# PhilippBongartz/RepeatResolver

Measured on AMD Instinct MI355X. Metric: sum-of-pairs DP cells/sec, higher is better.
Workload: dtype u32

## Files before the change

repeatresolver_amd/csrc/pwr_device.hip:

```cpp
#include <hip/hip_runtime.h>

#include <algorithm>
#include <chrono>
#include <cstdint>
#include <cstdio>
#include <cstdlib>
#include <cstring>
#include <new>
#include <thread>
#include <type_traits>
#include <vector>

#include "pwr.h"

#define PWR_INF 0x40000000u
#define PWR_BIG 0x7fffffff

struct Hdr {
    int W;
    int nslots;
    int nfree;
    int cur;
    int status;
    int stop;
// ... 193 lines not shown
}

template <int NT>
__device__ __forceinline__ unsigned block_incl_add(unsigned v, unsigned *sh, unsigned &total)
{
    const int lane = threadIdx.x & 63, wave = threadIdx.x >> 6;
    unsigned incl = wave_incl_add(v);
    if (lane == 63) sh[wave] = incl;
    __syncthreads();
    unsigned wp = 0, tot = 0;
#pragma unroll
    for (int w = 0; w < NT / 64; ++w) {
        unsigned s = sh[w];
        wp += (w < wave) ? s : 0u;
        tot += s;
    }
    __syncthreads();
    total = tot;
    return incl + wp;
}

template <int NT>
__device__ __forceinline__ unsigned block_min_u32(unsigned v, unsigned *sh)
{
    for (int o = 32; o > 0; o >>= 1) v = min(v, (unsigned)__shfl_xor((int)v, o));
    if ((threadIdx.x & 63) == 0) sh[threadIdx.x >> 6] = v;
    __syncthreads();
    unsigned r = 0xffffffffu;
#pragma unroll
    for (int w = 0; w < NT / 64; ++w) r = min(r, sh[w]);
    __syncthreads();
    return r;
}
template <int NT>
__device__ __forceinline__ int block_max_i32(int v, int *sh)
{
    for (int o = 32; o > 0; o >>= 1) v = max(v, __shfl_xor(v, o));
    if ((threadIdx.x & 63) == 0) sh[threadIdx.x >> 6] = v;
    __syncthreads();
    int r = INT_MIN;
#pragma unroll
    for (int w = 0; w < NT / 64; ++w) r = max(r, sh[w]);
    __syncthreads();
    return r;
}

__device__ __forceinline__ const int *cur_order(const DState &st)
{
    return st.hdr->cur ? st.order1 : st.order0;
}

#define GATHER_NT 1024
#define GATHER_G 16
struct GatherPart { unsigned long long ucost, cells; unsigned sum4, maxS, lastcov, tag; };

__device__ __forceinline__ int gather_row_of(const Hdr *hd, const int *bplan, int job, int *boff_out)
{
    int boff = 0;
    if (bplan[0] && job < PLAN_MAX) boff = bplan[1 + job];
    else {
        const unsigned long long ah = hd->ahead;
        int cnt = -1;
        for (boff = 0; boff < 64; ++boff) if (!((ah >> boff) & 1ull) && ++cnt == job) break;
        if (boff == 64) boff = 64 + (job - cnt - 1);
    }
    *boff_out = boff;
    const int kk = hd->next_row + boff;
    if (hd->status != 0 || hd->need_grow || job >= hd->nb || kk >= hd->row_end) return -1;
    return kk;
}

__global__ __launch_bounds__(GATHER_NT) void k_gather_a(DState st, JobBufs jb, const int *jobrows)
{
    const int job = blockIdx.x, g = blockIdx.y, tid = threadIdx.x;
    JobMeta *m = &jb.meta[job];
    const Hdr *hd = st.hdr;
    int boff;
    const int kk = gather_row_of(hd, st.bplan, job, &boff);
    if (g == 0) {
        const int nj = (int)gridDim.x;
        if (tid == 0) { CommitJob z; z.nchg = z.nev = z.ndel = 0; z.first = 0x7fffffff; z.u0 = z.u1 = 0; z.scanned = 0; z.pad = 0; jb.cjob[job] = z; jb.chkdone[job] = 0; }
        for (int j = tid; j < nj; j += GATHER_NT) { jb.pair_cf[(size_t)job * nj + j] = 0; jb.pair_left[(size_t)job * nj + j] = 0; }
    }
    if (kk < 0) { if (tid == 0 && g == 0) m->active = 0; return; }
    const int k = jobrows[kk];
    const int L = st.rowlen[k];
    const int W = hd->W;
    if (L == 0) {
        if (tid == 0 && g == 0) { m->k = k; m->L = 0; m->ok = 1; m->W = W; m->nnew = 0; m->cells = 0; m->ver = hd->version; m->active = 1; m->off = boff; m->wide = 0; m->abort = 0; }
        return;
    }
    const long long off = st.rowoff[k];
    const int *order = cur_order(st);
    int *way = jb.way + (size_t)job * jb.Lmax;
    const int B = st.B, H = st.H;
    const int way0 = st.rank[st.pos[off]], wayL = st.rank[st.pos[off + L - 1]];
    const int a0 = max(0, way0 - H), aL = max(0, wayL - H);
    const int lo = max(0, a0 - 1), hi = min(W - 1, aL + B - 1);
    const int n = hi - lo + 1;
    if (g == 0 && tid < 64 && hd->jumpmask != 0ull) {
        bool bad = false;
        if (tid > boff && ((hd->jumpmask >> tid) & 1ull)) {
            const int kkj = hd->next_row + tid;
            const int kj = jobrows[kkj], Lj = st.rowlen[kj];
            const long long oj = st.rowoff[kj];
            const int f = st.rank[st.pos[oj]], l = st.rank[st.pos[oj + Lj - 1]];
            const int *rec = st.bplan + JR_BASE + 4 * (kkj & 63);
            const int es = (int)((unsigned)hd->events_total - (unsigned)rec[0]);
            bad = !(hi + 2 < f - rec[1] - es || l + rec[2] + es < lo - 2);
        }
        if (__ballot(bad) != 0ull && tid == 0) atomicCAS(&st.hdr->status, 0, PWR_ERR_ORDER);
    }
    const int x0 = (int)((long long)L * g / GATHER_G), x1 = (int)((long long)L * (g + 1) / GATHER_G);
    uint8_t *mark = jb.mark + (size_t)job * jb.colcap;
    const int c0 = g == 0 ? lo : st.rank[st.pos[off + min(x0, L - 1)]], c1 = (g == GATHER_G - 1 || x1 >= L) ? hi + 1 : st.rank[st.pos[off + x1]];
    (void)n;
    for (int i = c0 - lo + tid; i < c1 - lo; i += GATHER_NT) mark[i] = 0;
    __syncthreads();
    unsigned long long mycells = 0;
    uint4 *desc = jb.desc + (size_t)job * jb.Lmax;
    const int NWg = jb.wpNW, MSg = jb.wpMS;
// ... 253 lines not shown
    unsigned carry = s_carry, maxS = 0;
    if (tid == 0) s_cov[0] = s_covl;
    __syncthreads();
    int it2 = 0;
    for (int base = i0; base < i1; base += GATHER_NT, ++it2) {
        const int i = base + tid;
        const bool valid = i < i1;
        const int y = lo + i;
        uint32_t w[6] = {0, 0, 0, 0, 0, 0};
        if (it2 < GC_K) {
#pragma unroll
            for (int k = 0; k < GC_K; ++k)
                if (it2 == k) {
#pragma unroll
                    for (int b = 0; b < 6; ++b) w[b] = cw[k][b];
                }
        } else if (valid) tally_of(y, w, &ucost);
        unsigned tot;
        const unsigned gin = block_incl_add<GATHER_NT>(w[4], sh, tot);
        s_cov[tid + 1] = w[5];
        __syncthreads();
        const unsigned covl = s_cov[tid];
        __syncthreads();
        if (tid == GATHER_NT - 1) s_cov[0] = w[5];
        if (valid) {
            const unsigned upc = (y == 0 || y == W - 1) ? PWR_INF : max(w[5], covl);
            const int gq = (int)(carry + gin);
            rec2[2 * i] = make_int4((int)w[0] - gq, (int)w[1] - gq, (int)w[2] - gq, (int)w[3] - gq);
            rec2[2 * i + 1] = make_int4((int)(upc == PWR_INF ? PWR_INF - 1u : upc) - gq, gq, (int)PWR_INF - gq, 0);
            maxS = max(maxS, max(max(w[0], w[1]), max(max(w[2], w[3]), max(w[4], w[5]))));
        }
        carry += tot;
        __syncthreads();
    }
    const unsigned mx = (unsigned)(~block_min_u32<GATHER_NT>(~maxS, sh));
    for (int o = 32; o > 0; o >>= 1) ucost += __shfl_xor(ucost, o);
    if ((tid & 63) == 0) s_u[tid >> 6] = ucost;
    __syncthreads();
    if (tid == 0) {
        unsigned long long U = 0;
        for (int w = 0; w < GATHER_NT / 64; ++w) U += s_u[w];
        __hip_atomic_store(&part[g].ucost, U, __ATOMIC_RELAXED, __HIP_MEMORY_SCOPE_AGENT);
        __hip_atomic_store(&part[g].maxS, mx, __ATOMIC_RELAXED, __HIP_MEMORY_SCOPE_AGENT);
        __hip_atomic_store(&part[g].lastcov, tag, __ATOMIC_RELEASE, __HIP_MEMORY_SCOPE_AGENT);
    }
    if (g == GATHER_G - 1 && tid < 64) {
        unsigned long long Ut = 0, cs = 0;
        unsigned mxt = 0;
        if (tid < GATHER_G) {
            while (__hip_atomic_load(&part[tid].lastcov, __ATOMIC_ACQUIRE, __HIP_MEMORY_SCOPE_AGENT) != tag) __builtin_amdgcn_s_sleep(1);
            Ut = __hip_atomic_load(&part[tid].ucost, __ATOMIC_RELAXED, __HIP_MEMORY_SCOPE_AGENT);
            mxt = __hip_atomic_load(&part[tid].maxS, __ATOMIC_RELAXED, __HIP_MEMORY_SCOPE_AGENT);
            cs = part[tid].cells;
        }
        for (int o = 32; o > 0; o >>= 1) { Ut += __shfl_xor(Ut, o); cs += __shfl_xor(cs, o); mxt = max(mxt, (unsigned)__shfl_xor((int)mxt, o)); }
        if (tid == 0) {
            const unsigned long long bound = Ut + (unsigned long long)mxt * (unsigned long long)(2 * B + 4096);
            m->maxS = mxt; m->cells = cs;
            m->wide = (jb.force64 || !(bound < (unsigned long long)PWR_INF && carry < (1u << 29))) ? 1 : 0;
            if (m->wide) st.hdr->need64 = 65;
        }
    }
}

#define V2_D 128
#define V2_PD 512
#define V2_R 64
#define V2_SPINS 256
#define FBIG 0x3fffffff
#define UNI(v) __builtin_amdgcn_readfirstlane(v)

__device__ __forceinline__ unsigned acc_push(unsigned acc, unsigned long long mask)
{
    unsigned long long carry_out;
    asm("v_addc_co_u32_e64 %0, %1, %0, %0, %2" : "+v"(acc), "=s"(carry_out) : "s"(mask));
    return acc;
}
#define ICMP_SGE 39
#define ICMP_SLE 41

#define V2_LOAD(MSX, SLOT, AU, AG, AI, GL)                                                       \
    {                                                                                            \
        _Pragma("unroll") for (int i = 0; i < C; ++i) {                                          \
            const int y_ = lo + (MSX) * MS + lc + i;                                             \
            int4 p_ = make_int4(PWR_BIG / 2, PWR_BIG / 2, PWR_BIG / 2, PWR_BIG / 2);             \
            int4 q_ = make_int4(PWR_BIG / 2, 0, PWR_BIG / 2, 0);                                 \
            if (y_ <= hi) { p_ = rec2[2 * (y_ - lo)]; q_ = rec2[2 * (y_ - lo) + 1]; }            \
            ldsS[wave][SLOT][0][lc + i] = p_.x; ldsS[wave][SLOT][1][lc + i] = p_.y;              \
            ldsS[wave][SLOT][2][lc + i] = p_.z; ldsS[wave][SLOT][3][lc + i] = p_.w;              \
            AU[i] = q_.x; AG[i] = q_.y; AI[i] = q_.z;                                            \
        }                                                                                        \
        const int yq_ = lo + (MSX) * MS - 1;                                                     \
        GL = (yq_ >= lo && yq_ <= hi) ? UNI(rec2[2 * (yq_ - lo) + 1].y) : 0;                     \
    }

template <int NW, int C>
__global__ __launch_bounds__(NW * 64) void k_fill_v2(DState st, JobBufs jb)
{
    constexpr int MS = 64 * C, RS = NW * MS;
    constexpr int MBDUMP = NW * V2_D, PTDUMP = V2_PD;
    __shared__ unsigned long long mbQ[2 * (MBDUMP + NW * 64)];
    __shared__ unsigned long long ptQ[PTDUMP + NW * 64];
    __shared__ __attribute__((aligned(16))) int ldsS[NW][2][4][MS];
    __shared__ int rdone[NW];
    __shared__ int s_done;
#define LD64(REF) __hip_atomic_load(&(REF), __ATOMIC_RELAXED, __HIP_MEMORY_SCOPE_WORKGROUP)
// ... 2753 lines not shown
#define HIPC(call)                                                                     \
    do {                                                                               \
        hipError_t e_ = (call);                                                        \
        if (e_ != hipSuccess) {                                                        \
            fprintf(stderr, "pwr: %s failed: %s\n", #call, hipGetErrorString(e_));    \
            return PWR_ERR_DEVICE;                                                     \
        }                                                                              \
    } while (0)

struct pwr_ctx {
    int T = 0, B = 0, H = 0, device = 0;
    int W_host = 0;
    std::vector<unsigned char> text;
    bool on_device = false;
    DState st{};
    JobBufs jb{};
    int njobs = 0;
    int *d_jobrows = nullptr;
    int *d_rowids = nullptr;
    std::vector<int> ids, pos_lo;
    unsigned long long *d_score = nullptr;
    hipStream_t stream = nullptr;
    std::vector<int> rowlen;
    long long sumL = 0;
    int Lmax = 0;
    int window = 3;
    double batch_ema = 1.0;
    int profile = 0;
    unsigned gather_tag = 0;
    int force64 = 0;
    int evcap = EVCAP;
    int stall_test = 0;
    int par_trace = 2;
    int cap_slack = 8192;
    int spec_len = 6;
    int fill_mode = 4;
    double host_enqueue_s = 0, host_wait_s = 0;
    unsigned host_seq = 0;
    int seen_fallback = 0, seen_need64 = 0;
    unsigned trace_epoch = 0;
    unsigned fill_epoch = 0;
    int wave_cols = 0;
    int wp_waves = 5;
    int one_wg = 0;
    int one_wg_lds = 0;
    int fill_lds = 0;
    int seg_rows = 160;
    int seg_align = 16;
    int seg_max = 64;
    int seg_budget = 0;
    int seg_minrows = 64;
    int spec_inorder = 64, plan_gate_rel = 1, plan_len = 0;
    int check_in_trace = 1;
    int fail_stops = 1, hard_rows = 1, hard_up_pm = 300, hard_down_pm = 0;
    int plan_slack = PLAN_SLACK, plan_evrate_x100 = (int)(PLAN_EVRATE_MAX * 100.0f);
    int plan_ahead = 1;
    int seg_balance = 0;
    int split_rank = 0, split_world = 1;
    int split_k0 = 0, split_kend = 0;
    int src_start = 1;
    int warm_pct = 190;
    int warm_adapt = 1;
    int warm_min_pct = 100;
    int warm_down_pm = 5, warm_up_pm = 50;
    pwr_stats stats{};
    std::vector<std::pair<hipEvent_t, hipEvent_t>> ev_pool;
    size_t ev_used = 0;
    void *h_hdr = nullptr;
    void *h_ring = nullptr;
    unsigned char *snap_dev = nullptr, *snap_host = nullptr;
    size_t snap_cap = 0;
    hipStream_t snap_stream = nullptr;
    hipEvent_t snap_taken = nullptr, snap_done = nullptr;
    bool snap_busy = false;
    std::vector<void *> allocs;
};
struct pwr_snapshot { pwr_ctx *c; int rows, width; size_t bytes; };

template <class F>
static void par_rows(int T, F f)
{
    unsigned nt = std::min<unsigned>(std::max(1u, std::thread::hardware_concurrency()), 16u);
    nt = (unsigned)std::max(1, std::min<int>((int)nt, T / 64));
    if (nt <= 1) { f(0, T, 0); return; }
    std::vector<std::thread> th;
    for (unsigned t = 0; t < nt; ++t)
        th.emplace_back([=]() { f((int)((long long)T * t / nt), (int)((long long)T * (t + 1) / nt), (int)t); });
    for (auto &x : th) x.join();
}
static unsigned par_threads(int T)
{
    unsigned nt = std::min<unsigned>(std::max(1u, std::thread::hardware_concurrency()), 16u);
    return (unsigned)std::max(1, std::min<int>((int)nt, T / 64));
}

static int code_of_char(unsigned char c)
{
    switch (c) {
    case 'a': case 'A': return 0;
    case 'c': case 'C': return 1;
    case 'g': case 'G': return 2;
    case 't': case 'T': return 3;
    case '-': case '_': return 4;
    case ' ': return 5;
    default: return -1;
    }
// ... 503 lines not shown
static int drain_events(pwr_ctx *c)
{
    if (!c->ev_used) return PWR_OK;
    HIPC(hipStreamSynchronize(c->stream));
    for (size_t i = 0; i < c->ev_used; ++i) {
        float ms = 0;
        HIPC(hipEventElapsedTime(&ms, c->ev_pool[i].first, c->ev_pool[i].second));
        c->stats.fill_ms += ms;
    }
    c->ev_used = 0;
    return PWR_OK;
}

static int ensure_device(pwr_ctx *c)
{
    if (c->on_device) { if (hipSetDevice(c->device) != hipSuccess) return PWR_ERR_DEVICE; return PWR_OK; }
    int rc = upload(c);
    if (rc) { free_device(c); return rc; }
    return PWR_OK;
}

static void stats_from_hdr(pwr_ctx *c, const Hdr &h)
{
    c->stats.cells_computed = h.cells_computed;
    c->stats.cells_reference = h.cells_reference;
    c->stats.rows_changed = h.rows_changed;
    c->stats.batches = h.batches;
    c->stats.rows_committed = h.rows_committed;
    c->stats.rows_recomputed = h.rows_recomputed;
    c->stats.rows_wide = h.rows_wide;
    c->stats.stalls = h.stalls;
    c->stats.rows_ahead = h.rows_ahead;
    c->stats.seg_jobs = h.seg_jobs; c->stats.segs = h.segs; c->stats.seg_fails = h.seg_fails;
    c->stats.rows_jumped = h.rows_jumped;
    for (int i = 0; i < 4; ++i) c->stats.reject_reason[i] = h.fail_reason[i];
}

static int check_status(pwr_ctx *c)
{
    Hdr h;
    int rc = read_hdr(c, &h);
    if (rc) return rc;
    stats_from_hdr(c, h);
    return h.status;
}

static int enqueue_front(pwr_ctx *c)
{
    const int n = c->window;
    int rc;
    c->jb.gather_tag = ++c->gather_tag;
    c->jb.rowids = c->d_rowids;
    c->jb.f64_follows = (c->seen_need64 > 0 || c->force64) ? 1 : 0;
    hipLaunchKernelGGL(k_gather_a, dim3(n, GATHER_G), dim3(GATHER_NT), 0, c->stream, c->st, c->jb, c->d_rowids);
    hipLaunchKernelGGL(k_gather_c, dim3(n, GATHER_G + 1), dim3(GATHER_NT), 0, c->stream, c->st, c->jb);
    c->jb.trace_ny = (c->jb.Lmax / TB_C + TB_W) / TB_W;
    c->jb.check_in_trace = (c->check_in_trace && c->fill_mode == 4 && c->par_trace == 2 && c->st.colcap < TB_MAXCOL && c->jb.smax > 1 && c->jb.seg_rows > 0) ? 1 : 0;
    if ((rc = launch_fill(c, n))) return rc;
    if (c->jb.f64_follows) hipLaunchKernelGGL(k_fill64, dim3(n), dim3(F64_NT), 0, c->stream, c->st, c->jb);
    if (c->par_trace) {
        if (++c->trace_epoch >= (1u << 14)) { HIPC(hipMemsetAsync(c->jb.gtr, 0, (size_t)c->njobs * c->jb.trk * 8, c->stream)); c->trace_epoch = 1; }
        c->jb.trace_tag = c->trace_epoch;
        c->jb.trace_blk = (c->par_trace == 2 && c->st.colcap < TB_MAXCOL) ? 1 : 0;
        if (c->jb.trace_blk) hipLaunchKernelGGL(k_trace_blk, dim3(n, c->jb.trace_ny + (c->jb.check_in_trace ? c->jb.smax - 1 : 0)), dim3(TB_W * 64), 0, c->stream, c->st, c->jb);
        else hipLaunchKernelGGL(k_trace_par, dim3(n, TRK / TRW), dim3(TRW * 64), 0, c->stream, c->st, c->jb);
    }
    else { c->jb.trace_blk = 0; hipLaunchKernelGGL(k_trace_wp, dim3(n), dim3(64), 0, c->stream, c->st, c->jb); }
    HIPC(hipGetLastError());
    return PWR_OK;
}

static int enqueue_commit(pwr_ctx *c, Hdr *host_copy, unsigned host_seq)
{
    const int n = c->window;
    hipLaunchKernelGGL(k_commit_scan, dim3(n, CS_G), dim3(COMMIT_NT), 0, c->stream, c->st, c->jb, n);
    hipLaunchKernelGGL(k_commit_apply, dim3(CA_G), dim3(COMMIT_NT), 0, c->stream, c->st, c->jb, n);
    hipLaunchKernelGGL(k_commit_finish, dim3(CA_G), dim3(COMMIT_NT), 0, c->stream, c->st, c->jb, n, c->d_rowids, host_copy, host_seq);
    HIPC(hipGetLastError());
    return PWR_OK;
}

static int enqueue_batch(pwr_ctx *c, Hdr *host_copy, unsigned host_seq)
{
    int rc = enqueue_front(c);
    if (rc) return rc;
    return enqueue_commit(c, host_copy, host_seq);
}

#define PWR_INFLIGHT 3
#define PWR_POLL_LIMIT_S 120

static int slab_init(pwr_ctx *c, int k0, int n)
{
    const int kend = k0 + n;
    int nb = (int)(c->batch_ema + 2.6);
    nb = std::max(1, std::min(nb, std::min(c->window, n)));
    for (int j = 1; j < nb; ++j)
        if (c->rowlen[c->ids[k0 + j]] > c->rowlen[c->ids[k0]] + (int)((long long)c->rowlen[c->ids[k0]] * c->spec_len / 100) + 64) { nb = j; break; }
    const float ema0 = (float)c->batch_ema;
    struct { int next_row, row_end, nb, need_grow, window; } init = {k0, kend, nb, 0, c->window};
    static_assert(sizeof(init) == offsetof(Hdr, fallback) - offsetof(Hdr, next_row), "slab fields of Hdr");
    HIPC(hipMemcpyAsync(&c->st.hdr->ema, &ema0, sizeof(float), hipMemcpyHostToDevice, c->stream));
    HIPC(hipMemcpyAsync(&c->st.hdr->speclen, &c->spec_len, sizeof(int), hipMemcpyHostToDevice, c->stream));
    HIPC(hipMemcpyAsync(&c->st.hdr->next_row, &init, sizeof init, hipMemcpyHostToDevice, c->stream));
    HIPC(hipMemsetAsync(&c->st.hdr->ahead, 0, sizeof(unsigned long long), c->stream));
    HIPC(hipMemsetAsync(c->st.bplan, 0, sizeof(int), c->stream));
    HIPC(hipMemsetAsync(&c->st.hdr->jumpmask, 0, sizeof(unsigned long long), c->stream));
    HIPC(hipStreamSynchronize(c->stream));
// ... 292 lines not shown
extern "C" int pwr_snapshot_wait(pwr_snapshot *sn, const unsigned char **image, size_t *bytes, int *rows, int *width)
{
    if (!sn || !sn->c) return PWR_ERR_ARG;
    if (hipSetDevice(sn->c->device) != hipSuccess) return PWR_ERR_DEVICE;
    if (sn->bytes > 0) HIPC(hipEventSynchronize(sn->c->snap_done));
    if (image) *image = sn->c->snap_host;
    if (bytes) *bytes = sn->bytes;
    if (rows) *rows = sn->rows;
    if (width) *width = sn->width;
    return PWR_OK;
}

extern "C" void pwr_snapshot_free(pwr_snapshot *sn)
{
    if (!sn) return;
    if (sn->c && sn->bytes > 0 && sn->c->snap_done) { (void)hipSetDevice(sn->c->device); (void)hipEventSynchronize(sn->c->snap_done); }
    if (sn->c) sn->c->snap_busy = false;
    delete sn;
}

extern "C" int pwr_trim_ends(pwr_ctx *c)
{
    if (!c) return PWR_ERR_ARG;
    if (!c->on_device) { host_trim(c); return PWR_OK; }
    return PWR_OK;
}

extern "C" int pwr_set_option(pwr_ctx *c, const char *key, long value)
{
    if (!c || !key) return PWR_ERR_ARG;
    if (!strcmp(key, "window")) { if (value < 1 || value > 128 || c->on_device) return PWR_ERR_ARG; c->window = (int)value; return PWR_OK; }
    if (!strcmp(key, "profile")) { if (value < 0 || value > 1000000) return PWR_ERR_ARG; c->profile = (int)value; return PWR_OK; }
    if (!strcmp(key, "spec_len")) { if (value < 0 || value > 100000) return PWR_ERR_ARG; c->spec_len = (int)value; return PWR_OK; }
    if (!strcmp(key, "fill")) { if (c->on_device || (value != 3 && value != 4)) return PWR_ERR_ARG; c->fill_mode = (int)value; return PWR_OK; }
    if (!strcmp(key, "stall_test")) { if (value < 0 || value > 1000000) return PWR_ERR_ARG; c->stall_test = (int)value; return PWR_OK; }
    if (!strcmp(key, "evcap")) { if (value < 0 || value > EVCAP) return PWR_ERR_ARG; c->evcap = (int)value; c->jb.evcap = (int)value; return PWR_OK; }
    if (!strcmp(key, "force64")) { if (value != 0 && value != 1) return PWR_ERR_ARG; c->force64 = (int)value; c->jb.force64 = (int)value; return PWR_OK; }
    if (!strcmp(key, "ptrace")) { if (value < 0 || value > 2) return PWR_ERR_ARG; c->par_trace = (int)value; return PWR_OK; }
    if (!strcmp(key, "slack")) { if (c->on_device || value < 0) return PWR_ERR_ARG; c->cap_slack = (int)value; return PWR_OK; }
    if (!strcmp(key, "fill_epoch")) { if (value < 0 || value >= (1 << 15)) return PWR_ERR_ARG; c->fill_epoch = (unsigned)value; return PWR_OK; }
    if (!strcmp(key, "trace_epoch")) { if (value < 0 || value >= (1 << 14)) return PWR_ERR_ARG; c->trace_epoch = (unsigned)value; return PWR_OK; }
    if (!strcmp(key, "onewg")) { if (value != 0 && value != 1) return PWR_ERR_ARG; c->one_wg = (int)value; return PWR_OK; }
    if (!strcmp(key, "fill_lds")) { if (value < 0 || value > 100000) return PWR_ERR_ARG; c->fill_lds = (int)value; return PWR_OK; }
    if (!strcmp(key, "onewg_lds")) { if (value < 0 || value > 100000) return PWR_ERR_ARG; c->one_wg_lds = (int)value; return PWR_OK; }
    if (!strcmp(key, "seg_rows")) { if (c->on_device || value < 0 || value > 1000000) return PWR_ERR_ARG; c->seg_rows = (int)value; return PWR_OK; }
    if (!strcmp(key, "seg_align")) { if (c->on_device || (value != 16 && value != 32 && value != 64)) return PWR_ERR_ARG; c->seg_align = (int)value; return PWR_OK; }
    if (!strcmp(key, "seg_max")) { if (c->on_device || value < 1 || value > SEG_MAX) return PWR_ERR_ARG; c->seg_max = (int)value; return PWR_OK; }
    if (!strcmp(key, "seg_budget")) { if (value < 0 || value > 100000) return PWR_ERR_ARG; c->seg_budget = (int)value; c->jb.seg_budget = (int)value; return PWR_OK; }
    if (!strcmp(key, "plan_slack")) { if (value < 0 || value > 1000000) return PWR_ERR_ARG; c->plan_slack = (int)value; c->jb.plan_slack = (int)value; return PWR_OK; }
    if (!strcmp(key, "hard_rows")) { if (c->on_device || value < 0 || value > 2) return PWR_ERR_ARG; c->hard_rows = (int)value; return PWR_OK; }
    if (!strcmp(key, "hard_up_pm")) { if (c->on_device || value < 1 || value > 100000) return PWR_ERR_ARG; c->hard_up_pm = (int)value; return PWR_OK; }
    if (!strcmp(key, "hard_down_pm")) { if (c->on_device || value < 0 || value > 100000) return PWR_ERR_ARG; c->hard_down_pm = (int)value; return PWR_OK; }
    if (!strcmp(key, "check_in_trace")) { if (value < 0 || value > 1) return PWR_ERR_ARG; c->check_in_trace = (int)value; return PWR_OK; }
    if (!strcmp(key, "plan_len")) { if (value < 0 || value > 100000) return PWR_ERR_ARG; c->plan_len = (int)value; c->jb.plan_len = (int)value; return PWR_OK; }
    if (!strcmp(key, "plan_gate_rel")) { if (value < 0 || value > 1) return PWR_ERR_ARG; c->plan_gate_rel = (int)value; c->jb.plan_gate_rel = (int)value; return PWR_OK; }
    if (!strcmp(key, "spec_inorder")) { if (value < 0 || value > 64) return PWR_ERR_ARG; c->spec_inorder = (int)value; c->jb.spec_inorder = (int)value; return PWR_OK; }
    if (!strcmp(key, "fail_stops")) { if (value < 0 || value > 1) return PWR_ERR_ARG; c->fail_stops = (int)value; c->jb.fail_stops = (int)value; return PWR_OK; }
    if (!strcmp(key, "plan_evrate_x100")) { if (value < 0 || value > 100000000) return PWR_ERR_ARG; c->plan_evrate_x100 = (int)value; c->jb.plan_evrate_x100 = (int)value; return PWR_OK; }
    if (!strcmp(key, "plan_ahead")) { if (value != 0 && value != 1) return PWR_ERR_ARG; c->plan_ahead = (int)value; c->jb.plan_ahead = (int)value; return PWR_OK; }
    if (!strcmp(key, "seg_balance")) { if (value != 0 && value != 1) return PWR_ERR_ARG; c->seg_balance = (int)value; c->jb.seg_balance = (int)value; return PWR_OK; }
    if (!strcmp(key, "seg_minrows")) { if (value < 16 || value > 100000) return PWR_ERR_ARG; c->seg_minrows = (int)value; c->jb.seg_minrows = (int)value; return PWR_OK; }
    if (!strcmp(key, "src_start")) { if (c->on_device || value < 0 || value > 1) return PWR_ERR_ARG; c->src_start = (int)value; return PWR_OK; }
    if (!strcmp(key, "warm_adapt")) { if (c->on_device || value < 0 || value > 1) return PWR_ERR_ARG; c->warm_adapt = (int)value; return PWR_OK; }
    if (!strcmp(key, "warm_down_pm")) { if (c->on_device || value < 1 || value > 1000) return PWR_ERR_ARG; c->warm_down_pm = (int)value; return PWR_OK; }
    if (!strcmp(key, "warm_up_pm")) { if (c->on_device || value < 1 || value > 10000) return PWR_ERR_ARG; c->warm_up_pm = (int)value; return PWR_OK; }
    if (!strcmp(key, "warm_min_pct")) { if (c->on_device || value < 0 || value > 100000) return PWR_ERR_ARG; c->warm_min_pct = (int)value; return PWR_OK; }
    if (!strcmp(key, "warm_pct")) { if (c->on_device || value < 0 || value > 100000) return PWR_ERR_ARG; c->warm_pct = (int)value; return PWR_OK; }
    if (!strcmp(key, "wave_cols")) { if (c->on_device || (value != 0 && value != 4)) return PWR_ERR_ARG; c->wave_cols = (int)value; return PWR_OK; }
    if (!strcmp(key, "waves")) { if (c->on_device || (value != 3 && value != 4 && value != 5 && value != 8 && value != 9 && value != 17)) return PWR_ERR_ARG; c->wp_waves = (int)value; return PWR_OK; }
    return PWR_ERR_ARG;
}

extern "C" int pwr_get_option(pwr_ctx *c, const char *key, long *value)
{
    if (!c || !key || !value) return PWR_ERR_ARG;
    if (!strcmp(key, "window")) *value = c->window;
    else if (!strcmp(key, "profile")) *value = c->profile;
    else if (!strcmp(key, "spec_len")) *value = c->spec_len;
    else if (!strcmp(key, "fill")) *value = c->fill_mode;
    else if (!strcmp(key, "ptrace")) *value = c->par_trace;
    else if (!strcmp(key, "force64")) *value = c->force64;
    else if (!strcmp(key, "slack")) *value = c->cap_slack;
    else if (!strcmp(key, "waves")) *value = c->wp_waves;
    else if (!strcmp(key, "onewg")) *value = c->one_wg;
    else if (!strcmp(key, "seg_rows")) *value = c->seg_rows;
    else if (!strcmp(key, "seg_max")) *value = c->seg_max;
    else if (!strcmp(key, "seg_budget")) *value = c->seg_budget;
    else if (!strcmp(key, "seg_minrows")) *value = c->seg_minrows;
    else if (!strcmp(key, "seg_balance")) *value = c->seg_balance;
    else if (!strcmp(key, "plan_ahead")) *value = c->plan_ahead;
    else if (!strcmp(key, "plan_slack")) *value = c->plan_slack;
    else if (!strcmp(key, "plan_evrate_x100")) *value = c->plan_evrate_x100;
    else if (!strcmp(key, "fail_stops")) *value = c->fail_stops;
    else if (!strcmp(key, "spec_inorder")) *value = c->spec_inorder;
    else if (!strcmp(key, "plan_gate_rel")) *value = c->plan_gate_rel;
    else if (!strcmp(key, "plan_len")) *value = c->plan_len;
    else if (!strcmp(key, "check_in_trace")) *value = c->check_in_trace;
    else if (!strcmp(key, "hard_rows")) *value = c->hard_rows;
    else if (!strcmp(key, "hard_up_pm")) *value = c->hard_up_pm;
    else if (!strcmp(key, "hard_down_pm")) *value = c->hard_down_pm;
    else if (!strcmp(key, "hard_marked") || !strcmp(key, "hard_fills") || !strcmp(key, "hard_refail")) {
        *value = 0;
        if (c->on_device) { Hdr h; int rc = read_hdr(c, &h); if (rc) return rc; *value = (long)(key[5] == 'm' ? h.hard_marked : key[5] == 'f' ? h.hard_fills : h.hard_refail); }
    }
    else if (!strcmp(key, "evrate_x100")) {
        *value = 0;
        if (c->on_device) { Hdr h; int rc = read_hdr(c, &h); if (rc) return rc; *value = (long)(h.evrate * 100.0f); }
    }
    else if (!strcmp(key, "warm_pct")) *value = c->warm_pct;
    else if (!strcmp(key, "src_start")) *value = c->src_start;
    else if (!strcmp(key, "warm_adapt")) *value = c->warm_adapt;
    else if (!strcmp(key, "host_enqueue_us")) *value = (long)(c->host_enqueue_s * 1e6);
    else if (!strcmp(key, "host_wait_us")) *value = (long)(c->host_wait_s * 1e6);
    else if (!strcmp(key, "warm_now")) {
        if (!c->on_device) *value = c->warm_pct;
        else { Hdr h; int rc = read_hdr(c, &h); if (rc) return rc; *value = h.warm_step > 0 ? (long)(((long long)h.warm_cur * 100 + c->B / 2) / c->B) : c->warm_pct; }
    }
    else if (!strcmp(key, "warm_min_pct")) *value = c->warm_min_pct;
    else if (!strcmp(key, "warm_down_pm")) *value = c->warm_down_pm;
    else if (!strcmp(key, "warm_up_pm")) *value = c->warm_up_pm;
    else return PWR_ERR_ARG;
    return PWR_OK;
}

extern "C" int pwr_get_stats(pwr_ctx *c, pwr_stats *out)
{
    if (!c || !out) return PWR_ERR_ARG;
    if (c->on_device) {
        if (hipSetDevice(c->device) != hipSuccess) return PWR_ERR_DEVICE;
        int rc = check_status(c);
        if (rc) return rc;
        if ((rc = drain_events(c))) return rc;
    }
    *out = c->stats;
    return PWR_OK;
}

extern "C" int pwr_reset_stats(pwr_ctx *c)
{
    if (!c) return PWR_ERR_ARG;
    if (c->on_device) {
        if (hipSetDevice(c->device) != hipSuccess) return PWR_ERR_DEVICE;
        int rc0 = drain_events(c);
        if (rc0) return rc0;
    }
    c->stats = pwr_stats{};
    if (c->on_device) {
        if (hipSetDevice(c->device) != hipSuccess) return PWR_ERR_DEVICE;
        HIPC(hipStreamSynchronize(c->stream));
        HIPC(hipMemset(&c->st.hdr->cells_computed, 0, 16 * sizeof(unsigned long long)));
// ... 79 lines not shown
```

Baseline: 53.33 billion.

## Fuse gather_a and gather_c into one kernel with inter-block flag handoff

Replaces the two gather kernel launches with a single fused kernel. Each block prefetches its tally words into registers before writing the way, mark and descriptor arrays. It then signals completion through a per-partition waytag, and an extra block per job waits on those tags before planning segments. The goal is to remove one launch and the kernel boundary between the two phases, and to overlap the tally loads with the descriptor work. In exchange it depends on inter-block spin-waits that assume all blocks are co-resident, and it lets rows proceed when the order error was raised inside the same kernel.

Measured after the change: 53.46 billion (median of 6 runs). No clear change (+0.2%).

```diff
diff --git a/repeatresolver_amd/csrc/pwr_device.hip b/repeatresolver_amd/csrc/pwr_device.hip
--- a/repeatresolver_amd/csrc/pwr_device.hip
+++ b/repeatresolver_amd/csrc/pwr_device.hip
@@ -269,9 +269,12 @@
 
 #define GATHER_NT 1024
 #define GATHER_G 16
-struct GatherPart { unsigned long long ucost, cells; unsigned sum4, maxS, lastcov, tag; };
-
-__device__ __forceinline__ int gather_row_of(const Hdr *hd, const int *bplan, int job, int *boff_out)
+struct GatherPart {
+    unsigned long long ucost, cells; unsigned sum4, maxS, lastcov, tag;
+    unsigned waytag, pad;
+};
+
+__device__ __forceinline__ int gather_row_of(const Hdr *hd, const int *bplan, int job, int *boff_out, bool raised_here = false)
 {
     int boff = 0;
     if (bplan[0] && job < PLAN_MAX) boff = bplan[1 + job];
@@ -283,7 +286,8 @@
     }
     *boff_out = boff;
     const int kk = hd->next_row + boff;
-    if (hd->status != 0 || hd->need_grow || job >= hd->nb || kk >= hd->row_end) return -1;
+    const int status = hd->status;
+    if ((status != 0 && !(raised_here && status == PWR_ERR_ORDER)) || hd->need_grow || job >= hd->nb || kk >= hd->row_end) return -1;
     return kk;
 }
 
@@ -643,6 +647,259 @@
             Ut = __hip_atomic_load(&part[tid].ucost, __ATOMIC_RELAXED, __HIP_MEMORY_SCOPE_AGENT);
             mxt = __hip_atomic_load(&part[tid].maxS, __ATOMIC_RELAXED, __HIP_MEMORY_SCOPE_AGENT);
             cs = part[tid].cells;
+        }
+        for (int o = 32; o > 0; o >>= 1) { Ut += __shfl_xor(Ut, o); cs += __shfl_xor(cs, o); mxt = max(mxt, (unsigned)__shfl_xor((int)mxt, o)); }
+        if (tid == 0) {
+            const unsigned long long bound = Ut + (unsigned long long)mxt * (unsigned long long)(2 * B + 4096);
+            m->maxS = mxt; m->cells = cs;
+            m->wide = (jb.force64 || !(bound < (unsigned long long)PWR_INF && carry < (1u << 29))) ? 1 : 0;
+            if (m->wide) st.hdr->need64 = 65;
+        }
+    }
+}
+
+__device__ __forceinline__ void gather_way_done(GatherPart *part, int g, unsigned tag)
+{
+    asm volatile("s_waitcnt vmcnt(0)" ::: "memory");
+    __syncthreads();
+    if (threadIdx.x == 0) __hip_atomic_store(&part[g].waytag, tag, __ATOMIC_RELEASE, __HIP_MEMORY_SCOPE_AGENT);
+}
+
+__global__ __launch_bounds__(GATHER_NT) void k_gather(DState st, JobBufs jb, const int *jobrows)
+{
+    __shared__ unsigned sh[GATHER_NT / 64];
+    __shared__ unsigned s_cov[GATHER_NT + 1];
+    __shared__ unsigned long long s_u[GATHER_NT / 64], s_cells[GATHER_NT / 64];
+    __shared__ unsigned s_carry, s_covl;
+    __shared__ int s_lblank;
+    const int job = blockIdx.x, g = blockIdx.y, tid = threadIdx.x;
+    GatherPart *part = jb.gpart + (size_t)job * GATHER_G;
+    const unsigned tag = jb.gather_tag;
+    if (g == GATHER_G) {
+        if (tid < GATHER_G)
+            while (__hip_atomic_load(&part[tid].waytag, __ATOMIC_ACQUIRE, __HIP_MEMORY_SCOPE_AGENT) != tag) __builtin_amdgcn_s_sleep(1);
+        __syncthreads();
+        plan_segments(st, jb, job);
+        return;
+    }
+    JobMeta *m = &jb.meta[job];
+    const Hdr *hd = st.hdr;
+    int boff;
+    const int kk = gather_row_of(hd, st.bplan, job, &boff, true);
+    if (g == 0) {
+        const int nj = (int)gridDim.x;
+        if (tid == 0) { CommitJob z; z.nchg = z.nev = z.ndel = 0; z.first = 0x7fffffff; z.u0 = z.u1 = 0; z.scanned = 0; z.pad = 0; jb.cjob[job] = z; jb.chkdone[job] = 0; }
+        for (int j = tid; j < nj; j += GATHER_NT) { jb.pair_cf[(size_t)job * nj + j] = 0; jb.pair_left[(size_t)job * nj + j] = 0; }
+    }
+    if (kk < 0) { if (tid == 0 && g == 0) m->active = 0; gather_way_done(part, g, tag); return; }
+    const int k = jobrows[kk];
+    const int L = st.rowlen[k];
+    const int W = hd->W;
+    if (L == 0) {
+        if (tid == 0 && g == 0) { m->k = k; m->L = 0; m->ok = 1; m->W = W; m->nnew = 0; m->cells = 0; m->ver = hd->version; m->active = 1; m->off = boff; m->wide = 0; m->abort = 0; }
+        gather_way_done(part, g, tag);
+        return;
+    }
+    const long long off = st.rowoff[k];
+    const int *order = cur_order(st);
+    int *way = jb.way + (size_t)job * jb.Lmax;
+    const int B = st.B, H = st.H;
+    const int way0 = st.rank[st.pos[off]], wayL = st.rank[st.pos[off + L - 1]];
+    const int a0 = max(0, way0 - H), aL = max(0, wayL - H);
+    const int lo = max(0, a0 - 1), hi = min(W - 1, aL + B - 1);
+    if (g == 0 && tid < 64 && hd->jumpmask != 0ull) {
+        bool bad = false;
+        if (tid > boff && ((hd->jumpmask >> tid) & 1ull)) {
+            const int kkj = hd->next_row + tid;
+            const int kj = jobrows[kkj], Lj = st.rowlen[kj];
+            const long long oj = st.rowoff[kj];
+            const int f = st.rank[st.pos[oj]], l = st.rank[st.pos[oj + Lj - 1]];
+            const int *rec = st.bplan + JR_BASE + 4 * (kkj & 63);
+            const int es = (int)((unsigned)hd->events_total - (unsigned)rec[0]);
+            bad = !(hi + 2 < f - rec[1] - es || l + rec[2] + es < lo - 2);
+        }
+        if (__ballot(bad) != 0ull && tid == 0) atomicCAS(&st.hdr->status, 0, PWR_ERR_ORDER);
+    }
+    const int x0 = (int)((long long)L * g / GATHER_G), x1 = (int)((long long)L * (g + 1) / GATHER_G);
+    uint8_t *mark = jb.mark + (size_t)job * jb.colcap;
+    const int c0 = g == 0 ? lo : st.rank[st.pos[off + min(x0, L - 1)]], c1 = (g == GATHER_G - 1 || x1 >= L) ? hi + 1 : st.rank[st.pos[off + x1]];
+    const int i0 = c0 - lo, i1 = c1 - lo;
+    constexpr int GC_K = 6;
+    uint32_t cw[GC_K][6];
+#pragma unroll
+    for (int it = 0; it < GC_K; ++it) {
+        const int i = i0 + tid + it * GATHER_NT;
+#pragma unroll
+        for (int b = 0; b < 6; ++b) cw[it][b] = 0;
+        if (i < i1) {
+            const Tally t = st.tally[order[lo + i]];
+#pragma unroll
+            for (int b = 0; b < 6; ++b) cw[it][b] = t.w[b];
+        }
+    }
+    if (tid == 0) s_lblank = 0;
+    unsigned long long mycells = 0;
+    uint4 *desc = jb.desc + (size_t)job * jb.Lmax;
+    const int NWg = jb.wpNW, MSg = jb.wpMS;
+    for (int x = x0 + tid; x < x1; x += GATHER_NT) {
+        const int wx = st.rank[st.pos[off + x]];
+        const int wn = x + 1 < L ? st.rank[st.pos[off + x + 1]] : wx + 1;
+        way[x] = wx;
+        mark[wx - lo] = (uint8_t)(st.seq[off + x] + 1);
+        for (int y = wx + 1; y < wn; ++y) mark[y - lo] = 0;
+        const int ax = max(0, wx - H), bx = min(B, W - ax);
+        mycells += (unsigned long long)bx;
+        const int mlo = (ax - lo) / MSg, mhi = (ax + bx - 1 - lo) / MSg;
+        int ap = 0, bp = 0, plo = 0, phi = -1;
+        if (x > 0) {
+            ap = max(0, st.rank[st.pos[off + x - 1]] - H); bp = min(B, W - ap);
+            plo = (ap - lo) / MSg; phi = (ap + bp - 1 - lo) / MSg;
+        }
+        unsigned long long fl = 0;
+        unsigned fl2 = 0;
+        for (int w = 0; w < NWg; ++w) {
+            const int msw = mlo + (((w - mlo) % NWg) + NWg) % NWg;
+            if (msw > mhi) continue;
+            const int msp = plo + (((w - plo) % NWg) + NWg) % NWg;
+            const bool ranp = x > 0 && msp == msw && msp <= phi;
+            const int yq = lo + msw * MSg - 1;
+            const unsigned kind = (x == 0 || yq < ap) ? 0u : (yq < ap + bp ? 1u : 2u);
+            const unsigned bits = ((ranp && x < L - 1 && kind != 2u) ? 1u : 0u) | (msw > mlo ? 2u : 0u) | (kind == 1u ? 4u : 0u) | (msw == mhi ? 8u : 0u);
+            if (w < 16) fl |= (unsigned long long)bits << (4 * w); else fl2 |= bits << (4 * (w - 16));
+        }
+        desc[x] = make_uint4((unsigned)ax | ((unsigned)st.seq[off + x] << 24), (unsigned)fl, (unsigned)(fl >> 32), fl2);
+    }
+    if (g == 0) for (int i = tid; i < way0 - lo; i += GATHER_NT) mark[i] = 0;
+    if (g == GATHER_G - 1) for (int i = wayL + 1 - lo + tid; i <= hi - lo; i += GATHER_NT) mark[i] = 0;
+    {
+        const int nbk = st.nbrk[k];
+        if (nbk > 0) {
+            const int *bxs = st.brkx + st.brkoff[k];
+            __syncthreads();
+            for (int t = tid; t < nbk; t += GATHER_NT) {
+                const int b = bxs[t];
+                if (b >= x0 && b < x1)
+                    for (int y = st.rank[st.pos[off + b]] + 1; y < st.rank[st.pos[off + b + 1]]; ++y) mark[y - lo] = 7;
+                if (b == x0 - 1 && st.rank[st.pos[off + b]] + 1 < c0) s_lblank = 1;
+            }
+        }
+    }
+    for (int o = 32; o > 0; o >>= 1) mycells += __shfl_xor(mycells, o);
+    if ((tid & 63) == 0) s_cells[tid >> 6] = mycells;
+    if (tid == 0 && g == 0) {
+        m->k = k; m->L = L; m->lo = lo; m->hi = hi; m->W = W; m->entry = -1; m->nnew = 0; m->abort = 0; m->active = 1; m->off = boff;
+        m->ver = hd->version; m->slot_lo = order[lo]; m->slot_hi = order[hi]; m->ok = 1; m->changed = 0;
+    }
+    gather_way_done(part, g, tag);
+    __threadfence_block();
+    auto take_own = [&](int y, uint32_t *w, unsigned long long *uc) {
+        if (y >= way0 && y <= wayL) {
+            const int mk = mark[y - lo];
+            const int own = mk == 7 ? 5 : (mk ? mk - 1 : 4);
+#pragma unroll
+            for (int b = 0; b < 6; ++b) w[b] -= (own != 5 && b != own) ? 1u : 0u;
+            if (uc) {
+#pragma unroll
+                for (int b = 0; b < 5; ++b) *uc += (b == own) ? w[b] : 0u;
+            }
+        }
+    };
+    auto tally_of = [&](int y, uint32_t *w, unsigned long long *uc) {
+        const Tally t = st.tally[order[y]];
+#pragma unroll
+        for (int b = 0; b < 6; ++b) w[b] = t.w[b];
+        take_own(y, w, uc);
+    };
+    unsigned mysum = 0;
+    unsigned long long ucost = 0;
+#pragma unroll
+    for (int it = 0; it < GC_K; ++it) {
+        const int i = i0 + tid + it * GATHER_NT;
+        if (i < i1) { take_own(lo + i, cw[it], &ucost); mysum += cw[it][4]; }
+    }
+    for (int i = i0 + tid + GC_K * GATHER_NT; i < i1; i += GATHER_NT) { uint32_t w[6]; tally_of(lo + i, w, nullptr); mysum += w[4]; }
+    for (int o = 32; o > 0; o >>= 1) mysum += __shfl_xor(mysum, o);
+    if ((tid & 63) == 0) sh[tid >> 6] = mysum;
+    __syncthreads();
+    if (tid == 0) {
+        unsigned tot = 0;
+        for (int w = 0; w < GATHER_NT / 64; ++w) tot += sh[w];
+        __hip_atomic_store(&part[g].sum4, tot, __ATOMIC_RELAXED, __HIP_MEMORY_SCOPE_AGENT);
+        __hip_atomic_store(&part[g].tag, tag, __ATOMIC_RELEASE, __HIP_MEMORY_SCOPE_AGENT);
+    }
+    if (tid < 64) {
+        unsigned mine = 0;
+        if (tid < g) {
+            while (__hip_atomic_load(&part[tid].tag, __ATOMIC_ACQUIRE, __HIP_MEMORY_SCOPE_AGENT) != tag) __builtin_amdgcn_s_sleep(1);
+            mine = __hip_atomic_load(&part[tid].sum4, __ATOMIC_RELAXED, __HIP_MEMORY_SCOPE_AGENT);
+        }
+        for (int o = 32; o > 0; o >>= 1) mine += __shfl_xor(mine, o);
+        if (tid == 0) s_carry = mine;
+    } else if (tid == 64) {
+        unsigned cl = 0;
+        if (i0 > 0) {
+            const int y = c0 - 1;
+            cl = st.tally[order[y]].w[5];
+            if (y >= way0 && y <= wayL && !s_lblank) cl -= 1u;
+        }
+        s_covl = cl;
+    }
+    __syncthreads();
+    unsigned carry = s_carry, maxS = 0;
+    if (tid == 0) s_cov[0] = s_covl;
+    __syncthreads();
+    int it2 = 0;
+    for (int base = i0; base < i1; base += GATHER_NT, ++it2) {
+        const int i = base + tid;
+        const bool valid = i < i1;
+        const int y = lo + i;
+        uint32_t w[6] = {0, 0, 0, 0, 0, 0};
+        if (it2 < GC_K) {
+#pragma unroll
+            for (int kq = 0; kq < GC_K; ++kq)
+                if (it2 == kq) {
+#pragma unroll
+                    for (int b = 0; b < 6; ++b) w[b] = cw[kq][b];
+                }
+        } else if (valid) tally_of(y, w, &ucost);
+        unsigned tot;
+        const unsigned gin = block_incl_add<GATHER_NT>(w[4], sh, tot);
+        s_cov[tid + 1] = w[5];
+        __syncthreads();
+        const unsigned covl = s_cov[tid];
+        __syncthreads();
+        if (tid == GATHER_NT - 1) s_cov[0] = w[5];
+        if (valid) {
+            const unsigned upc = (y == 0 || y == W - 1) ? PWR_INF : max(w[5], covl);
+            const int gq = (int)(carry + gin);
+            int4 *rec2 = jb.rec2 + (size_t)job * jb.colcap * 2;
+            rec2[2 * i] = make_int4((int)w[0] - gq, (int)w[1] - gq, (int)w[2] - gq, (int)w[3] - gq);
+            rec2[2 * i + 1] = make_int4((int)(upc == PWR_INF ? PWR_INF - 1u : upc) - gq, gq, (int)PWR_INF - gq, 0);
+            maxS = max(maxS, max(max(w[0], w[1]), max(max(w[2], w[3]), max(w[4], w[5]))));
+        }
+        carry += tot;
+        __syncthreads();
+    }
+    const unsigned mx = (unsigned)(~block_min_u32<GATHER_NT>(~maxS, sh));
+    for (int o = 32; o > 0; o >>= 1) ucost += __shfl_xor(ucost, o);
+    if ((tid & 63) == 0) s_u[tid >> 6] = ucost;
+    __syncthreads();
+    if (tid == 0) {
+        unsigned long long U = 0, cs = 0;
+        for (int w = 0; w < GATHER_NT / 64; ++w) { U += s_u[w]; cs += s_cells[w]; }
+        __hip_atomic_store(&part[g].ucost, U, __ATOMIC_RELAXED, __HIP_MEMORY_SCOPE_AGENT);
+        __hip_atomic_store(&part[g].cells, cs, __ATOMIC_RELAXED, __HIP_MEMORY_SCOPE_AGENT);
+        __hip_atomic_store(&part[g].maxS, mx, __ATOMIC_RELAXED, __HIP_MEMORY_SCOPE_AGENT);
+        __hip_atomic_store(&part[g].lastcov, tag, __ATOMIC_RELEASE, __HIP_MEMORY_SCOPE_AGENT);
+    }
+    if (g == GATHER_G - 1 && tid < 64) {
+        unsigned long long Ut = 0, cs = 0;
+        unsigned mxt = 0;
+        if (tid < GATHER_G) {
+            while (__hip_atomic_load(&part[tid].lastcov, __ATOMIC_ACQUIRE, __HIP_MEMORY_SCOPE_AGENT) != tag) __builtin_amdgcn_s_sleep(1);
+            Ut = __hip_atomic_load(&part[tid].ucost, __ATOMIC_RELAXED, __HIP_MEMORY_SCOPE_AGENT);
+            mxt = __hip_atomic_load(&part[tid].maxS, __ATOMIC_RELAXED, __HIP_MEMORY_SCOPE_AGENT);
+            cs = __hip_atomic_load(&part[tid].cells, __ATOMIC_RELAXED, __HIP_MEMORY_SCOPE_AGENT);
         }
         for (int o = 32; o > 0; o >>= 1) { Ut += __shfl_xor(Ut, o); cs += __shfl_xor(cs, o); mxt = max(mxt, (unsigned)__shfl_xor((int)mxt, o)); }
         if (tid == 0) {
@@ -3502,6 +3759,7 @@
     int seg_minrows = 64;
     int spec_inorder = 64, plan_gate_rel = 1, plan_len = 0;
     int check_in_trace = 1;
+    int gather_fused = 1;
     int fail_stops = 1, hard_rows = 1, hard_up_pm = 300, hard_down_pm = 0;
     int plan_slack = PLAN_SLACK, plan_evrate_x100 = (int)(PLAN_EVRATE_MAX * 100.0f);
     int plan_ahead = 1;
@@ -4111,8 +4369,11 @@
     c->jb.gather_tag = ++c->gather_tag;
     c->jb.rowids = c->d_rowids;
     c->jb.f64_follows = (c->seen_need64 > 0 || c->force64) ? 1 : 0;
-    hipLaunchKernelGGL(k_gather_a, dim3(n, GATHER_G), dim3(GATHER_NT), 0, c->stream, c->st, c->jb, c->d_rowids);
-    hipLaunchKernelGGL(k_gather_c, dim3(n, GATHER_G + 1), dim3(GATHER_NT), 0, c->stream, c->st, c->jb);
+    if (c->gather_fused) hipLaunchKernelGGL(k_gather, dim3(n, GATHER_G + 1), dim3(GATHER_NT), 0, c->stream, c->st, c->jb, c->d_rowids);
+    else {
+        hipLaunchKernelGGL(k_gather_a, dim3(n, GATHER_G), dim3(GATHER_NT), 0, c->stream, c->st, c->jb, c->d_rowids);
+        hipLaunchKernelGGL(k_gather_c, dim3(n, GATHER_G + 1), dim3(GATHER_NT), 0, c->stream, c->st, c->jb);
+    }
     c->jb.trace_ny = (c->jb.Lmax / TB_C + TB_W) / TB_W;
     c->jb.check_in_trace = (c->check_in_trace && c->fill_mode == 4 && c->par_trace == 2 && c->st.colcap < TB_MAXCOL && c->jb.smax > 1 && c->jb.seg_rows > 0) ? 1 : 0;
     if ((rc = launch_fill(c, n))) return rc;
@@ -4511,6 +4772,7 @@
     if (!strcmp(key, "hard_up_pm")) { if (c->on_device || value < 1 || value > 100000) return PWR_ERR_ARG; c->hard_up_pm = (int)value; return PWR_OK; }
     if (!strcmp(key, "hard_down_pm")) { if (c->on_device || value < 0 || value > 100000) return PWR_ERR_ARG; c->hard_down_pm = (int)value; return PWR_OK; }
     if (!strcmp(key, "check_in_trace")) { if (value < 0 || value > 1) return PWR_ERR_ARG; c->check_in_trace = (int)value; return PWR_OK; }
+    if (!strcmp(key, "gather_fused")) { if (value < 0 || value > 1) return PWR_ERR_ARG; c->gather_fused = (int)value; return PWR_OK; }
     if (!strcmp(key, "plan_len")) { if (value < 0 || value > 100000) return PWR_ERR_ARG; c->plan_len = (int)value; c->jb.plan_len = (int)value; return PWR_OK; }
     if (!strcmp(key, "plan_gate_rel")) { if (value < 0 || value > 1) return PWR_ERR_ARG; c->plan_gate_rel = (int)value; c->jb.plan_gate_rel = (int)value; return PWR_OK; }
     if (!strcmp(key, "spec_inorder")) { if (value < 0 || value > 64) return PWR_ERR_ARG; c->spec_inorder = (int)value; c->jb.spec_inorder = (int)value; return PWR_OK; }
@@ -4555,6 +4817,7 @@
     else if (!strcmp(key, "plan_gate_rel")) *value = c->plan_gate_rel;
     else if (!strcmp(key, "plan_len")) *value = c->plan_len;
     else if (!strcmp(key, "check_in_trace")) *value = c->check_in_trace;
+    else if (!strcmp(key, "gather_fused")) *value = c->gather_fused;
     else if (!strcmp(key, "hard_rows")) *value = c->hard_rows;
     else if (!strcmp(key, "hard_up_pm")) *value = c->hard_up_pm;
     else if (!strcmp(key, "hard_down_pm")) *value = c->hard_down_pm;
```
